# shichaoy/pop_up_slam

Measured on AMD Instinct MI355X. Metric: graph-solve iters/sec + final chi2, 1k-pose/5k-edge plane graph, higher is better.
Workload: dtype f64; 1 GPU; C2 synthetic corridor: 1000 SE3 poses, 200 planes, 5000 plane edges, 999 odometry edges (BASELINE.json configs[1], seed 42); jacobian_mode=numeric, total_lm_solves=773

## Files before the change

### pop_up_slam_amd/csrc/pps_k3.hip

```cpp
#include <algorithm>
#include <atomic>
#include <cstdlib>

#include <hip/hip_ext.h>

#include "pps_kcommon.h"
#include "pps_regtile.h"
#include "pps_front_reg.h"

namespace pps {



int lds_front_limit() {
  int fa = 1;
  while ((size_t)(fa + 1) * ((fa + 1) | 1) * 8 <= (size_t)kLdsLaunchCeilingBytes) fa++;
  return fa - 1;
}

template <bool USE_LDS>
__global__ __launch_bounds__(256) void k_front_factor(DevGraph d, int level_begin, double lambda) {
  extern __shared__ double lds[];
  const int s = d.level_fronts[level_begin + blockIdx.x];
  const int p = d.f_p[s], b = d.f_b[s];
// ... 207 lines not shown
#pragma unroll
    for (int r = 0; r < 4; r++) {
      cok[t][r] = rok[r] && br <= I + lq + 4 * r;
      const double craw = F[cok[t][r] ? crt[r] + br : 0];
      c[t][r] = cok[t][r] ? craw : 0.0;
    }
  }
#pragma unroll
  for (int t = 0; t < NT; t++) c[t] = __builtin_amdgcn_mfma_f64_16x16x4f64(av, bv[t], c[t], 0, 0, 0);
#pragma unroll
  for (int t = 0; t < NT; t++) {
    const int cc = o + 16 * t + l16;
#pragma unroll
    for (int r = 0; r < 4; r++)
      if (cok[t][r]) F[crt[r] + cc] = c[t][r];
  }
}

__device__ __forceinline__ void wave_front_factor(const DevGraph& d, int s_in, double lambda, double* __restrict__ F) {
  const int lane = threadIdx.x & 63;
  const int s = uni(s_in);
  const int p = uni(d.f_p[s]), b = uni(d.f_b[s]);
  const int f = p + b, fa = f + 1;
  const int ntri = tri(fa);
  PPS_TR(0);
  for (int i = lane; i < ntri; i += 64) F[i] = 0.0;
  __builtin_amdgcn_wave_barrier();
  PPS_TR(1);
  {
    const int e0 = uni(d.f_el_off[s]), e1 = uni(d.f_el_off[s + 1]);
    const double damp = 1.0 + lambda;
    const int* __restrict__ tgp = d.el_tgt;
    const double* __restrict__ hf = d.Hf;
    for (int e = e0 + lane; e < e1; e += 64 * 8) {
      int tg[8]; double v[8];
#pragma unroll
      for (int u = 0; u < 8; u++) { const int x = e + 64 * u; tg[u] = x < e1 ? tgp[x] : -1; v[u] = x < e1 ? hf[x] : 0.0; }
#pragma unroll
      for (int u = 0; u < 8; u++)
        if (tg[u] >= 0) F[tg[u] & 0x3fffffff] += (tg[u] & (1 << 30)) ? v[u] * damp : v[u];
    }
  }
  __builtin_amdgcn_wave_barrier();
  PPS_TR(2);
  const int ci0 = uni(d.f_child_off[s]), ci1 = uni(d.f_child_off[s + 1]);
  for (int ci = ci0; ci < ci1; ci++) {
    const int c = uni(d.child[ci]);
    const int bc1 = uni(d.f_b[c]) + 1;
    const int n = tri(bc1);
    const double* __restrict__ Uc = d.U + uni64(d.f_Uoff[c]);
    const int* __restrict__ tgc = d.ea_tgt + uni64(d.f_ea_off[c]);
    for (int e = lane; e < n; e += 64 * 8) {
      int tg[8]; double v[8];
#pragma unroll
      for (int u = 0; u < 8; u++) { const int x = e + 64 * u; tg[u] = x < n ? tgc[x] : -1; v[u] = x < n ? Uc[x] : 0.0; }
#pragma unroll
      for (int u = 0; u < 8; u++)
        if (tg[u] >= 0) F[tg[u]] += v[u];
    }
    __builtin_amdgcn_wave_barrier();
  }
  PPS_TR(3);
  const int r0 = lane, r1 = lane + 64;
  const int t0 = tri(r0), t1 = tri(r1);
  long long cyc_panel = 0, cyc_trail = 0;
  for (int K = 0; K < p; K += 4) {
    const long long tk0 = d.trace ? clock64() : 0;
    double a0[4], a1[4];
#pragma unroll
    for (int m = 0; m < 4; m++) {
      const int c = K + m;
      const bool v0 = c < p && r0 >= c && r0 < fa, v1 = c < p && r1 >= c && r1 < fa;
      const double x0 = F[v0 ? t0 + c : 0], x1 = F[v1 ? t1 + c : 0];
      a0[m] = v0 ? x0 : 0.0;
      a1[m] = v1 ? x1 : 0.0;
    }
#pragma unroll
    for (int m = 0; m < 4; m++) {
      const int c = K + m;
      if (c < p) {
        const double dmm = (c < 64) ? readlane_d(a0[m], c) : readlane_d(a1[m], c - 64);
        double dinv = 0.0;
        if (dmm > 0.0) dinv = rsqrt_nr(dmm);
        else if (lane == 0) raise_status(&d.result_dev[2], 1.0);
        if (r0 >= c) a0[m] *= dinv;
        if (r1 >= c) a1[m] *= dinv;
#pragma unroll
        for (int n = m + 1; n < 4; n++) {
          const int cn = K + n;
          if (cn < p) {
            const double lnm = (cn < 64) ? readlane_d(a0[m], cn) : readlane_d(a1[m], cn - 64);
            if (r0 >= cn) a0[n] -= a0[m] * lnm;
            if (r1 >= cn) a1[n] -= a1[m] * lnm;
          }
        }
      }
    }
#pragma unroll
    for (int m = 0; m < 4; m++) {
      const int c = K + m;
      if (c < p) {
        if (r0 >= c && r0 < fa) F[t0 + c] = a0[m];
        if (r1 >= c && r1 < fa) F[t1 + c] = a1[m];
      }
    }
    __builtin_amdgcn_wave_barrier();
    const long long tk1 = d.trace ? clock64() : 0;
    const int o = K + 4 < p ? K + 4 : p;
    const int nb = o - K;
    for (int I = o; I < fa; I += 16) {
      const int nt = ((I - o) >> 4) + 1;
      switch (nt) {
        case 1: trailing_tile_row<1>(F, fa, o, I, K, nb, lane); break;
        case 2: trailing_tile_row<2>(F, fa, o, I, K, nb, lane); break;
        case 3: trailing_tile_row<3>(F, fa, o, I, K, nb, lane); break;
        case 4: trailing_tile_row<4>(F, fa, o, I, K, nb, lane); break;
        case 5: trailing_tile_row<5>(F, fa, o, I, K, nb, lane); break;
        case 6: trailing_tile_row<6>(F, fa, o, I, K, nb, lane); break;
        case 7: trailing_tile_row<7>(F, fa, o, I, K, nb, lane); break;
        default: trailing_tile_row<8>(F, fa, o, I, K, nb, lane); break;
      }
    }
    __builtin_amdgcn_wave_barrier();
    if (d.trace) { const long long tk2 = clock64(); cyc_panel += tk1 - tk0; cyc_trail += tk2 - tk1; }
  }
  PPS_TR(4);
  if (d.trace && lane == 0) { d.trace[(size_t)s * 8 + 6] = cyc_panel; d.trace[(size_t)s * 8 + 7] = cyc_trail; }
  double* __restrict__ Lp = d.L + uni64(d.f_Loff[s]);
  if (lane < p) {
    for (int i0 = 0; i0 < fa; i0 += 8) {
      double v[8];
#pragma unroll
      for (int u = 0; u < 8; u++) { const int i = i0 + u; v[u] = F[(i < fa && lane <= i) ? tri(i) + lane : 0]; }
#pragma unroll
      for (int u = 0; u < 8; u++) { const int i = i0 + u; if (i < fa && lane <= i) Lp[(size_t)i * p + lane] = v[u]; }
    }
  }
  double* __restrict__ Us = d.U + uni64(d.f_Uoff[s]);
  for (int i0 = p; i0 < fa; i0 += 8) {
    for (int j = p + lane; j < fa; j += 64) {
      double v[8];
#pragma unroll
      for (int u = 0; u < 8; u++) { const int i = i0 + u; v[u] = F[(i < fa && j <= i) ? tri(i) + j : 0]; }
#pragma unroll
      for (int u = 0; u < 8; u++) { const int i = i0 + u; if (i < fa && j <= i) Us[tri(i - p) + j - p] = v[u]; }
    }
  }
  PPS_TR(5);
}

constexpr int kEaDepth = 10;
__device__ __forceinline__ void xg_store(double* p, double v) { __hip_atomic_store(p, v, __ATOMIC_RELAXED, __HIP_MEMORY_SCOPE_AGENT); }
__device__ __forceinline__ double xg_load(const double* p) { return __hip_atomic_load(p, __ATOMIC_RELAXED, __HIP_MEMORY_SCOPE_AGENT); }
template <int N> struct ElBatch { int tg[N]; double v[N]; };
template <int N, bool XH = false>
__device__ __forceinline__ void el_issue(const int* __restrict__ tgp, const double* __restrict__ val, int e, int e1, int lane, ElBatch<N>& q) {
  const int last = e1 > 0 ? e1 - 1 : 0;
#pragma unroll
  for (int u = 0; u < N; u++) {
    const int x = e + lane + 64 * u, xc = x < e1 ? x : last;
    const int t = tgp[xc];
    double v;
    if constexpr (XH) v = xg_load(val + xc); else v = val[xc];
    q.tg[u] = x < e1 ? t : -1; q.v[u] = x < e1 ? v : 0.0;
  }
}
template <bool ORIG, int N>
__device__ __forceinline__ void el_apply(const ElBatch<N>& q, double damp, double* __restrict__ F, int tr) {
  if constexpr (ORIG) {
#pragma unroll
    for (int u = 0; u < N; u++) {
      const int t = q.tg[u] >= 0 ? (q.tg[u] & 0x3fffffff) : tr;
      F[t] = (q.tg[u] & (1 << 30)) && q.tg[u] >= 0 ? q.v[u] * damp : q.v[u];
    }
    return;
  }
  int t[N]; double old[N];
#pragma unroll
  for (int u = 0; u < N; u++) { t[u] = q.tg[u] >= 0 ? q.tg[u] : tr; old[u] = F[t[u]]; }
#pragma unroll
  for (int u = 0; u < N; u++) F[t[u]] = old[u] + q.v[u];
}
template <int NPRE> struct FrontPre { ElBatch<NPRE> q; int crv; };
template <int NPRE>
__device__ __forceinline__ void front_pre_issue(const DevGraph& d, int rec, int lane, FrontPre<NPRE>& o) {
  const int e0 = __builtin_amdgcn_readlane(rec, 3), e1 = __builtin_amdgcn_readlane(rec, 4);
  const int cr0 = __builtin_amdgcn_readlane(rec, 5), nch = __builtin_amdgcn_readlane(rec, 6);
  el_issue(d.el_tgt, d.Hf, e0, e1, lane, o.q);
  o.crv = (lane < 8 * nch) ? d.crec[(size_t)cr0 * 8 + lane] : 0;
}
__device__ __forceinline__ void front_clear(int rec, int lane, double* __restrict__ F) {
  const int ntri = tri(__builtin_amdgcn_readlane(rec, 1) + __builtin_amdgcn_readlane(rec, 2) + 1);
  double2* __restrict__ F2 = reinterpret_cast<double2*>(F);
  const int n2 = ntri >> 1;
#pragma unroll 4
  for (int i = lane; i < n2; i += 64) F2[i] = make_double2(0.0, 0.0);
  if (lane == 0) F[ntri - 1] = 0.0;
  __builtin_amdgcn_wave_barrier();
}
template <int NPRE>
__device__ __forceinline__ void front_pre_finish(const DevGraph& d, int rec, int lane, const FrontPre<NPRE>& o, double damp, double* __restrict__ F, int tr) {
  const int e0 = __builtin_amdgcn_readlane(rec, 3), e1 = __builtin_amdgcn_readlane(rec, 4);
  el_apply<true>(o.q, damp, F, tr);
  for (int e = e0 + 64 * NPRE; e < e1; e += 64 * 8) { ElBatch<8> q; el_issue(d.el_tgt, d.Hf, e, e1, lane, q); __builtin_amdgcn_wave_barrier(); el_apply<true>(q, damp, F, tr); }
  __builtin_amdgcn_wave_barrier();
}
struct XGroup { int* flag; int epoch; double* hand; };
constexpr size_t kXgLdsFloorBytes = 82 * 1024;
__device__ __forceinline__ void xg_post(const XGroup& x, int s) {
  asm volatile("s_waitcnt vmcnt(0)" ::: "memory");
  if ((threadIdx.x & 63) == 0) __hip_atomic_store(x.flag + s, x.epoch, __ATOMIC_RELAXED, __HIP_MEMORY_SCOPE_AGENT);
}
template <bool ACQ>
__device__ __forceinline__ void xg_wait(const DevGraph& d, const XGroup& x, int s) {
  int spin = 0;
  while (__hip_atomic_load(x.flag + s, __ATOMIC_RELAXED, __HIP_MEMORY_SCOPE_AGENT) != x.epoch) {
    if (++spin >= (1 << 21)) { if ((threadIdx.x & 63) == 0) raise_status(&d.result_dev[2], kStatusInternal); break; }
    __builtin_amdgcn_s_sleep(2);
  }
  if (ACQ) __builtin_amdgcn_fence(__ATOMIC_ACQUIRE, "agent"); else __builtin_amdgcn_fence(__ATOMIC_ACQUIRE, "wavefront");
}
template <bool XG = false>
__device__ __forceinline__ void front_extend_add(const DevGraph& d, int rec, int crv0, int lane, double* __restrict__ F, int tr, const XGroup* xg = nullptr) {
  const int cr0 = __builtin_amdgcn_readlane(rec, 5), nch = __builtin_amdgcn_readlane(rec, 6);
  for (int cb = 0; cb < nch; cb += 8) {
    const int crv = cb == 0 ? crv0 : ((lane < 8 * (nch - cb)) ? d.crec[(size_t)(cr0 + cb) * 8 + lane] : 0);
    auto child = [&](int cj, int& n, const double* __restrict__& Uc, const int* __restrict__& tgc) {
      n = __builtin_amdgcn_readlane(crv, 8 * cj);
      const long long uo = ((long long)__builtin_amdgcn_readlane(crv, 8 * cj + 2) << 32) | (unsigned int)__builtin_amdgcn_readlane(crv, 8 * cj + 1);
      const long long eo = ((long long)__builtin_amdgcn_readlane(crv, 8 * cj + 4) << 32) | (unsigned int)__builtin_amdgcn_readlane(crv, 8 * cj + 3);
      Uc = d.U + uo; tgc = d.ea_tgt + eo;
    };
    int cj = 0;
    for (; cj < 8 && cb + cj < nch; cj++) {
      int n; const double* Uc; const int* tgc;
      child(cj, n, Uc, tgc);
      if (XG && __builtin_amdgcn_readlane(crv, 8 * cj + 6)) {
        xg_wait<false>(d, *xg, __builtin_amdgcn_readlane(crv, 8 * cj + 5));
        for (int e = 0; e < n; e += 64 * kEaDepth) { ElBatch<kEaDepth> q; el_issue<kEaDepth, true>(tgc, Uc, e, n, lane, q); __builtin_amdgcn_wave_barrier(); el_apply<false>(q, 0.0, F, tr); }
      } else
      for (int e = 0; e < n; e += 64 * kEaDepth) { ElBatch<kEaDepth> q; el_issue(tgc, Uc, e, n, lane, q); __builtin_amdgcn_wave_barrier(); el_apply<false>(q, 0.0, F, tr); }
      __builtin_amdgcn_wave_barrier();
    }
  }
}

constexpr int kPanelWBand = 4;
constexpr int kPanelWLevel = 8;
constexpr int kPanelWWide = 8;
template <bool TR>
__device__ __forceinline__ void front_assemble(const DevGraph& d, int rec, double lambda, double* F, int tr) {
  const int lane = threadIdx.x & 63;
  const int s = __builtin_amdgcn_readlane(rec, 0);
  (void)s;
  if (TR) PPS_TR(0);
  FrontPre<8> pre;
  front_pre_issue(d, rec, lane, pre);
  front_clear(rec, lane, F);
  if (TR) PPS_TR(1);
  front_pre_finish(d, rec, lane, pre, 1.0 + lambda, F, tr);
  if (TR) PPS_TR(2);
  front_extend_add(d, rec, pre.crv, lane, F, tr);
  if (TR) PPS_TR(3);
}
template <int NT, bool TR, bool STRIP = false, int W = kPanelWBand, bool XH = false>
__device__ __forceinline__ void front_eliminate_out(const DevGraph& d, int rec, double* F, double* P) {
  front_reg_eliminate<NT, TR, STRIP, W, XH>(d, rec, F, P);
}
template <int NT, bool TR, bool STRIP = false, int W = kPanelWBand>
__device__ __forceinline__ void wave_front_factor_reg(const DevGraph& d, int rec, double lambda, double* F, double* P, int tr) {
  front_assemble<TR>(d, rec, lambda, F, tr);
  front_eliminate_out<NT, TR, STRIP, W>(d, rec, F, P);
}

template <int K> __device__ __forceinline__ double row_bcast_d(double v) {
  int lo = __double2loint(v), hi = __double2hiint(v);
  lo = __builtin_amdgcn_update_dpp(0, lo, 0x150 + K, 0xf, 0xf, false);
  hi = __builtin_amdgcn_update_dpp(0, hi, 0x150 + K, 0xf, 0xf, false);
  return __hiloint2double(hi, lo);
}

constexpr double kFlowTimeout = kStatusInternal;
__device__ __forceinline__ void flow_wait(const DevGraph& d, int* flow, int q) {
  int spin = 0;
  while (__hip_atomic_load(flow + q, __ATOMIC_RELAXED, __HIP_MEMORY_SCOPE_WORKGROUP) == 0) {
    if (++spin >= (1 << 22)) { if ((threadIdx.x & 63) == 0) raise_status(&d.result_dev[2], kFlowTimeout); break; }
    __builtin_amdgcn_s_sleep(1);
  }
  __builtin_amdgcn_fence(__ATOMIC_ACQUIRE, "workgroup", "local");
}
__device__ __forceinline__ void flow_post(const DevGraph& d, int* flow, int slot, bool top) {
  __builtin_amdgcn_fence(__ATOMIC_RELEASE, "workgroup", "local");
  if ((threadIdx.x & 63) == 0 && !((d.sw & SW_DEBUG_DROP_FLAG) && top))
    __hip_atomic_store(flow + slot, 1, __ATOMIC_RELAXED, __HIP_MEMORY_SCOPE_WORKGROUP);
}

__device__ __forceinline__ bool xg_has_external_child(int rec, int crv, int lane) {
  const int nch = __builtin_amdgcn_readlane(rec, 6);
  return nch > 8 || __ballot((lane & 7) == 6 && lane < 8 * nch && crv != 0) != 0;
}
__device__ __forceinline__ void xg_publish(const XGroup& x, int s, int p, int b, int lane, double tj, double g0, double g1) {
  double* Xh = x.hand + (size_t)s * kBandMaxRows;
  if (lane < p) xg_store(Xh + lane, tj);
  if (lane < b) xg_store(Xh + p + lane, g0);
  if (lane + 64 < b) xg_store(Xh + p + lane + 64, g1);
  xg_post(x, s);
}

__device__ __forceinline__ void solve_pivot_scale(double (&lk)[16], double dinv) {
#define PPS_SC(U) lk[U] *= row_bcast_d<U>(dinv);
    PPS_SC(1) PPS_SC(2) PPS_SC(3) PPS_SC(4) PPS_SC(5) PPS_SC(6) PPS_SC(7) PPS_SC(8) PPS_SC(9) PPS_SC(10) PPS_SC(11) PPS_SC(12) PPS_SC(13) PPS_SC(14) PPS_SC(15)
#undef PPS_SC
}
template <bool SCALED = false>
__device__ __forceinline__ void solve_pivot_chain(int p, double (&lk)[16], double dinv, double& tj) {
#ifndef PPS_NO_FMA
#pragma clang fp contract(fast)
#endif
    if (!SCALED) solve_pivot_scale(lk, dinv);
#define PPS_BS(U) case U: tj -= lk[U] * row_bcast_d<U>(tj); [[fallthrough]];
    switch (p < 16 ? p - 1 : 15) {
      PPS_BS(15) PPS_BS(14) PPS_BS(13) PPS_BS(12) PPS_BS(11) PPS_BS(10) PPS_BS(9) PPS_BS(8)
      PPS_BS(7) PPS_BS(6) PPS_BS(5) PPS_BS(4) PPS_BS(3) PPS_BS(2)
      case 1: tj -= lk[1] * row_bcast_d<1>(tj); [[fallthrough]];
      default: break;
    }
#undef PPS_BS
    tj *= dinv;
}

template <bool GROUP = true, bool TR = false, bool XG = false>
__device__ __forceinline__ void wave_front_solve(const DevGraph& d, int rec, double* __restrict__ W, double* __restrict__ X, int slot, int* flow = nullptr, const XGroup* xg = nullptr) {
  const int lane = threadIdx.x & 63;
  const int s = __builtin_amdgcn_readlane(rec, 0);
  (void)s;
  if (TR) PPS_TR(0);
  const int p = __builtin_amdgcn_readlane(rec, 1), b = __builtin_amdgcn_readlane(rec, 2), f = p + b;
  const double* __restrict__ Lp = d.L + (((long long)__builtin_amdgcn_readlane(rec, 10) << 32) | (unsigned int)__builtin_amdgcn_readlane(rec, 9));
  const int pslot = GROUP ? __builtin_amdgcn_readlane(rec, 14) : -1;
  const int xpar = XG ? __builtin_amdgcn_readlane(rec, 13) : -1;
  int xcv = 0;
  if (XG) {
    const int nch = __builtin_amdgcn_readlane(rec, 6);
    const int* __restrict__ cp = nch > 0 ? d.crec + (size_t)__builtin_amdgcn_readlane(rec, 5) * 8 : d.frec;
    xcv = cp[lane < 8 * (nch < 8 ? nch : 8) ? lane : 0];
  }
  const int* __restrict__ ix = b == 0 ? d.frec : (pslot >= 0 || xpar >= 0 ? d.cmap + __builtin_amdgcn_readlane(rec, 15) : d.bidx + __builtin_amdgcn_readlane(rec, 8));
  double* xb = W;
  double* PL = W + kBandMaxRows;
  const int ix0r = ix[lane < b ? lane : 0], ix1r = ix[lane + 64 < b ? lane + 64 : 0];
  const int pix = d.pidx[__builtin_amdgcn_readlane(rec, 7) + (lane < p ? lane : 0)];
  const int n = (f + 1) * p;
  double tj = 0.0, dinv = 0.0;
  double lk[16];
  if (GROUP && p <= 16) {
#ifndef PPS_NO_FMA
#pragma clang fp contract(fast)
#endif
    const int j = lane & 15, part = lane >> 4;
    const int jc = j < p ? j : 0, lc = lane < p ? lane : 0;
    const double* __restrict__ LB = Lp + p * p + jc;
    const int blast = b > 0 ? b - 1 : 0;
    double lbv[12];
#pragma unroll
    for (int u = 0; u < 12; u++) { const int i = part + 4 * u; lbv[u] = LB[(i < b ? i : blast) * p]; }
#pragma unroll
    for (int u = 0; u < 16; u++) { const double l = Lp[(u < p ? u : p - 1) * p + lc]; lk[u] = lane < u ? l : 0.0; }
    const double dg = Lp[lc * p + lc], yr = Lp[f * p + jc];
    const int ix0 = lane < b ? ix0r : 0, ix1 = lane + 64 < b ? ix1r : 0;
    double g0 = 0.0, g1 = 0.0;
    const bool xpost = XG && xg_has_external_child(rec, xcv, lane);
    if (pslot < 0 && xpar < 0) { g0 = d.delta[ix0]; g1 = d.delta[ix1]; }
    if (flow) { dinv = 1.0 / dg; solve_pivot_scale(lk, dinv); }
    if (pslot >= 0) {
      if (flow) flow_wait(d, flow, pslot);
      const double* __restrict__ Xp = X + (size_t)pslot * kBandMaxRows; g0 = Xp[ix0]; g1 = Xp[ix1];
    } else if constexpr (XG) {
      if (xpar >= 0) {
        xg_wait<true>(d, *xg, xpar);
        const double* __restrict__ Xh = xg->hand + (size_t)xpar * kBandMaxRows; g0 = xg_load(Xh + ix0); g1 = xg_load(Xh + ix1);
      }
    }
    if (TR) PPS_TR(1);
    if (lane < b) xb[lane] = g0;
    if (lane + 64 < b) xb[lane + 64] = g1;
    __builtin_amdgcn_wave_barrier();
    if (TR) PPS_TR(2);
    if (!flow) dinv = 1.0 / dg;
    double a[4] = {part == 0 ? yr : 0.0, 0.0, 0.0, 0.0};
#pragma unroll
    for (int u = 0; u < 12; u++) { const int i = part + 4 * u; const double x = i < b ? xb[i] : 0.0; a[u & 3] -= lbv[u] * x; }
    for (int i0 = 48; i0 < b; i0 += 48) {
#pragma unroll
      for (int u = 0; u < 12; u++) { const int i = i0 + part + 4 * u; lbv[u] = LB[(i < b ? i : blast) * p]; }
// ... 83 lines not shown
      dinv = 1.0 / PL[lc * p + lc];
    }
    const int W = p <= 16 ? 16 : (p <= 32 ? 32 : 64), sh = p <= 16 ? 4 : (p <= 32 ? 5 : 6);
    const int j = lane & (W - 1), part = lane >> sh, np = 64 >> sh;
    const int jc = j < p ? j : 0;
    double a0 = (part == 0) ? (pre32 ? yq : PL[f * p + jc]) : 0.0, a1 = 0.0, a2 = 0.0, a3 = 0.0;
    const double* __restrict__ lb = PL + p * p + jc;
    int i_from = part;
    if (pre32) {
#pragma unroll
      for (int u = 0; u < 12; u += 4) {
        const int i = part + np * u, i1 = i + np, i2 = i + 2 * np, i3 = i + 3 * np;
        const double x0 = i < b ? xb[i] : 0.0, x1 = i1 < b ? xb[i1] : 0.0, x2 = i2 < b ? xb[i2] : 0.0, x3 = i3 < b ? xb[i3] : 0.0;
        if (i < b) { a0 -= lbq[u] * x0; a1 -= lbq[u + 1] * x1; a2 -= lbq[u + 2] * x2; a3 -= lbq[u + 3] * x3; }
      }
      i_from = part + 12 * np;
    }
    for (int i = i_from; i < b; i += 4 * np) {
      const int i1 = i + np, i2 = i + 2 * np, i3 = i + 3 * np;
      const double l0 = lb[i * p], l1 = lb[(i1 < b ? i1 : i) * p], l2 = lb[(i2 < b ? i2 : i) * p], l3 = lb[(i3 < b ? i3 : i) * p];
      const double x0 = xb[i], x1 = i1 < b ? xb[i1] : 0.0, x2 = i2 < b ? xb[i2] : 0.0, x3 = i3 < b ? xb[i3] : 0.0;
      a0 -= l0 * x0; a1 -= l1 * x1; a2 -= l2 * x2; a3 -= l3 * x3;
    }
    tj = (a0 + a1) + (a2 + a3);
    if (W <= 32) tj += __shfl_xor(tj, 32);
    if (W == 16) tj += __shfl_xor(tj, 16);
    tj = lane < p ? tj : 0.0;
    if (TR) PPS_TR(3);
    for (; k0 >= 16; k0 -= 16) {
#pragma unroll
      for (int u = 15; u >= 0; u--) {
        const int k = k0 + u;
        if (k < p) tj -= (pre_scaled ? lk[u] : lk[u] * readlane_d(dinv, k)) * readlane_d(tj, k);
      }
      pre_scaled = false;
#pragma unroll
      for (int u = 0; u < 16; u++) { const int k = k0 - 16 + u; const double l = PL[k * p + lc]; lk[u] = lane < k ? l : 0.0; }
    }
    solve_pivot_chain(p, lk, dinv, tj);
  }
  if (TR) PPS_TR(4);
  if (lane < p) d.delta[pix] = tj;
  if (TR) PPS_TR(5);
  if (!GROUP) return;
  double* __restrict__ Xs = X + (size_t)slot * kBandMaxRows;
  if (lane < p) Xs[lane] = tj;
  if (lane < b) Xs[p + lane] = g0;
  if (lane + 64 < b) Xs[p + lane + 64] = g1;
  if (flow) flow_post(d, flow, slot, pslot < 0);
  if (XG) { if (xpost) xg_publish(*xg, s, p, b, lane, tj, g0, g1); }
}

template <bool TR = false, bool XG = false>
__device__ __forceinline__ void body_band_solve_flow(const DevGraph& d, int g, int lds_doubles_per_wave, double* __restrict__ lds, int mg, const XGroup* xg = nullptr) {
  const int wave = uni(threadIdx.x >> 6), nw = blockDim.x >> 6;
  double* W = lds + (size_t)wave * lds_doubles_per_wave;
  double* X = lds + (size_t)nw * lds_doubles_per_wave;
  int* flow = reinterpret_cast<int*>(X + (size_t)mg * kBandMaxRows);
  const int2 span = reinterpret_cast<const int2*>(d.grp_span)[4 * (size_t)g];
  const int g0 = uni(span.x), gn = uni(span.y);
  const int i_first = g0 + gn - 1 - wave;
  int rec = i_first >= g0 ? d.frec[(size_t)i_first * 16 + (threadIdx.x & 15)] : 0;
  for (int q = threadIdx.x; q < gn; q += blockDim.x) flow[q] = 0;
  __syncthreads();
  for (int i = i_first; i >= g0; i -= nw) {
    wave_front_solve<true, TR, XG>(d, rec, W, X, i - g0, flow, xg);
    if (i - nw >= g0) rec = d.frec[(size_t)(i - nw) * 16 + (threadIdx.x & 15)];
  }
}
template <bool TR = false>
__device__ __forceinline__ void body_band_solve(const DevGraph& d, int g, int lds_doubles_per_wave, double* __restrict__ lds) {
  const int wave = uni(threadIdx.x >> 6), nw = blockDim.x >> 6;
  double* W = lds + (size_t)wave * lds_doubles_per_wave;
  double* X = lds + (size_t)nw * lds_doubles_per_wave;
  const int l0 = uni(d.grp_lvl_off[g]), l1 = uni(d.grp_lvl_off[g + 1]);
  int off[5], r4[4];
  {
    const int4 ga = reinterpret_cast<const int4*>(d.grp_span)[2 * (size_t)g], gb = reinterpret_cast<const int4*>(d.grp_span)[2 * (size_t)g + 1];
    off[0] = uni(ga.x); off[1] = uni(ga.w); off[2] = uni(gb.x); off[3] = uni(gb.y); off[4] = uni(gb.z);
  }
  const int g0 = off[0];
#pragma unroll
  for (int k = 0; k < 4; k++) { const int i = off[k] + wave; r4[k] = d.frec[(size_t)(i < off[k + 1] ? i : g0) * 16 + (threadIdx.x & 15)]; }
  for (int l = l1 - 1; l >= l0; l--) {
    const int k = l - l0;
    const int i0 = k < 4 ? (k == 3 ? off[3] : k == 2 ? off[2] : k == 1 ? off[1] : off[0]) : uni(d.glvl_front_off[l]);
    const int i1 = k < 4 ? (k == 3 ? off[4] : k == 2 ? off[3] : k == 1 ? off[2] : off[1]) : uni(d.glvl_front_off[l + 1]);
    for (int i = i0 + wave; i < i1; i += nw) {
      const int rec = (k < 4 && i == i0 + wave) ? (k == 3 ? r4[3] : k == 2 ? r4[2] : k == 1 ? r4[1] : r4[0]) : d.frec[(size_t)i * 16 + (threadIdx.x & 15)];
      wave_front_solve<true, TR>(d, rec, W, X, i - g0);
    }
    asm volatile("s_waitcnt lgkmcnt(0)\n\ts_barrier" ::: "memory");
  }
}

template <bool RESULT = true>
__device__ __forceinline__ void take_alt(DevGraph& d, const DualAlt& a) {
  if (blockIdx.y) { d.L = a.L; d.U = a.U; d.delta = a.delta; if (RESULT) d.result_dev = a.result_dev; }
}
__device__ __forceinline__ void take_alt(DevGraph& d, const DualAlt& a, double& lambda) {
  if (blockIdx.y) { d.L = a.L; d.U = a.U; d.delta = a.delta; d.result_dev = a.result_dev; lambda = a.lambda; }
}
__global__ __launch_bounds__(512) void k_band_solve(DevGraph d, DualAlt alt, int grp_begin, int lds_doubles_per_wave) {
  extern __shared__ double lds[];
  take_alt<false>(d, alt);
  body_band_solve(d, grp_begin + blockIdx.x, lds_doubles_per_wave, lds);
}
__global__ __launch_bounds__(768) void k_band_solve_flow(DevGraph d, DualAlt alt, int grp_begin, int lds_doubles_per_wave, int mg) {
  extern __shared__ double lds[];
  take_alt(d, alt);
  body_band_solve_flow(d, grp_begin + blockIdx.x, lds_doubles_per_wave, lds, mg);
}
__global__ __launch_bounds__(768) void k_band_solve_flow_trace(DevGraph d, int grp_begin, int lds_doubles_per_wave, int mg) {
  extern __shared__ double lds[];
  body_band_solve_flow<true>(d, grp_begin + blockIdx.x, lds_doubles_per_wave, lds, mg);
}
__global__ __launch_bounds__(512) void k_band_solve_trace(DevGraph d, int grp_begin, int lds_doubles_per_wave) {
  extern __shared__ double lds[];
  body_band_solve<true>(d, grp_begin + blockIdx.x, lds_doubles_per_wave, lds);
}

template <bool REG_ONLY, bool REG_STRIP = false, bool TR = false, bool R5 = false>
__device__ __forceinline__ void body_band_factor(const DevGraph& d, int g, double lambda, int lds_doubles_per_wave, double* __restrict__ lds) {
  const int wave = uni(threadIdx.x >> 6), nw = blockDim.x >> 6;
  double* F = lds + (size_t)wave * lds_doubles_per_wave;
  const int l0 = d.grp_lvl_off[g], l1 = d.grp_lvl_off[g + 1];
  const int4 ga = reinterpret_cast<const int4*>(d.grp_span)[2 * (size_t)g];
  for (int l = l0; l < l1; l++) {
    const int i1 = l == l0 ? ga.w : d.glvl_front_off[l + 1];
    for (int i = (l == l0 ? ga.x : d.glvl_front_off[l]) + wave; i < i1; i += nw) {
      const int rec = d.frec[(size_t)i * 16 + (threadIdx.x & 15)];
      const int s = __builtin_amdgcn_readlane(rec, 0);
      const int fa = __builtin_amdgcn_readlane(rec, 1) + __builtin_amdgcn_readlane(rec, 2) + 1;
      constexpr bool ALIAS = REG_ONLY && !REG_STRIP;
      double* const Pn = ALIAS ? F : F + lds_doubles_per_wave - kRegRowsMax * kP8Stride;
      const int tr = ALIAS ? lds_doubles_per_wave - 1 : lds_doubles_per_wave - kRegRowsMax * kP8Stride - 1;
      constexpr int WB = kPanelWBand, WR = kPanelWWide;
      if (REG_ONLY || fa <= kRegRowsMax) {
        if (REG_ONLY) front_assemble<TR>(d, rec, lambda, F, tr);
        else if ((fa <= kRegRowsMax && !d.no_strip) || fa <= kRegRows) front_assemble<true>(d, rec, lambda, F, tr);
      }
      if (REG_ONLY && fa <= 33) front_eliminate_out<2, TR, false, REG_STRIP ? WR : WB>(d, rec, F, Pn);
      else if (REG_ONLY && fa <= 49) front_eliminate_out<3, TR, false, REG_STRIP ? WR : WB>(d, rec, F, Pn);
      else if (REG_ONLY && (!REG_STRIP || fa <= kRegRows)) front_eliminate_out<4, TR, false, REG_STRIP ? WR : WB>(d, rec, F, Pn);
      else if (REG_ONLY && R5) front_eliminate_out<5, false, true, WR>(d, rec, F, Pn);
      else if (fa <= kRegRowsMax && !d.no_strip) front_eliminate_out<4, true, true, WR>(d, rec, F, Pn);
      else if (fa <= kRegRows) front_eliminate_out<4, true, false, WR>(d, rec, F, Pn);
      else wave_front_factor(d, s, lambda, F);
    }
    __syncthreads();
  }
}

template <int NPRE>
__device__ __forceinline__ int front_orig_entries(const DevGraph& d, int rec, int lane, double damp, double* F, int tr) {
  FrontPre<NPRE> pre;
  front_pre_issue(d, rec, lane, pre);
  front_clear(rec, lane, F);
  front_pre_finish(d, rec, lane, pre, damp, F, tr);
  return pre.crv;
}
__device__ __forceinline__ int front_orig_entries_sized(const DevGraph& d, int rec, int lane, double damp, double* F, int tr) {
  const int n_el = __builtin_amdgcn_readlane(rec, 4) - __builtin_amdgcn_readlane(rec, 3);
  if (n_el <= 192) return front_orig_entries<3>(d, rec, lane, damp, F, tr);
  return front_orig_entries<8>(d, rec, lane, damp, F, tr);
}

template <bool XG = false>
__device__ __forceinline__ void body_band_factor_pre(const DevGraph& d, int g, double lambda, int lds_doubles_per_wave, double* __restrict__ lds, const XGroup* xg = nullptr) {
  const int wave = uni(threadIdx.x >> 6), lane = threadIdx.x & 63, nw = uni(blockDim.x >> 6);
  const int4 ga = reinterpret_cast<const int4*>(d.grp_span)[2 * (size_t)g], gb = reinterpret_cast<const int4*>(d.grp_span)[2 * (size_t)g + 1];
  const int nl = uni(ga.z);
  const int o0 = uni(ga.x), o1 = uni(ga.w), o2 = uni(gb.x), o3 = uni(gb.y), o4 = uni(gb.z);
  const int n0 = o1 - o0, n1 = nl > 1 ? o2 - o1 : 0, n2 = nl > 2 ? o3 - o2 : 0, n3 = nl > 3 ? o4 - o3 : 0;
  double* F = lds + (size_t)wave * lds_doubles_per_wave;
  const int tr = lds_doubles_per_wave - 1;
  const bool shape_b = n0 + n1 + n2 + n3 <= nw;
  const int b1 = shape_b ? n0 : 0, b2 = shape_b ? n0 + n1 : n1, b3 = b2 + n2;
  int up_ll = 0, up_rec = 0;
  {
    int up_i = 0;
    if (shape_b && wave >= b1 && wave < b1 + n1) { up_ll = 1; up_i = o1 + wave - b1; }
    else if (wave >= b2 && wave < b2 + n2 && (shape_b || wave >= n1)) { up_ll = 2; up_i = o2 + wave - b2; }
    else if (wave >= b3 && wave < b3 + n3) { up_ll = 3; up_i = o3 + wave - b3; }
    if (up_ll) up_rec = d.frec[(size_t)up_i * 16 + (threadIdx.x & 15)];
  }
  const int pre_at = shape_b ? 0 : 1;
  int crv = 0;
  for (int ll = 0; ll < nl; ll++) {
    const int lb = ll == 0 ? 0 : ll == 1 ? b1 : ll == 2 ? b2 : b3;
    const int cnt = ll == 0 ? n0 : ll == 1 ? n1 : ll == 2 ? n2 : n3;
    const int i0 = ll == 0 ? o0 : ll == 1 ? o1 : ll == 2 ? o2 : o3;
    const bool mine = wave >= lb && wave < lb + cnt;
    const bool mine_up = mine && up_ll == ll && ll > pre_at;
    if (mine) {
      const int rec = (up_ll == ll && ll > 0) ? up_rec : d.frec[(size_t)(i0 + wave - lb) * 16 + (threadIdx.x & 15)];
      const int fa = __builtin_amdgcn_readlane(rec, 1) + __builtin_amdgcn_readlane(rec, 2) + 1;
      if (!mine_up) crv = front_orig_entries_sized(d, rec, lane, 1.0 + lambda, F, tr);
      front_extend_add<XG>(d, rec, crv, lane, F, tr, xg);
      if (fa <= 33) front_eliminate_out<2, false, false, kPanelWBand, XG>(d, rec, F, F);
      else if (fa <= 49) front_eliminate_out<3, false, false, kPanelWBand, XG>(d, rec, F, F);
      else front_eliminate_out<4, false, false, kPanelWBand, XG>(d, rec, F, F);
      if (XG) { if (__builtin_amdgcn_readlane(rec, 13) >= 0 && !(d.sw & SW_DEBUG_DROP_XFLAG)) xg_post(*xg, __builtin_amdgcn_readlane(rec, 0)); }
    } else if (ll == pre_at && up_ll > pre_at) {
      crv = front_orig_entries_sized(d, up_rec, lane, 1.0 + lambda, F, tr);
    }
    __syncthreads();
  }
}

template <bool REG_ONLY>
__global__ __launch_bounds__(512) void k_band_factor(DevGraph d, DualAlt alt, int grp_begin, double lambda, int lds_doubles_per_wave) {
  extern __shared__ double lds[];
  if (blockIdx.y) { d.L = alt.L; d.U = alt.U; d.delta = alt.delta; d.result_dev = alt.result_dev; lambda = alt.lambda; }
  body_band_factor<REG_ONLY>(d, grp_begin + blockIdx.x, lambda, lds_doubles_per_wave, lds);
}

template <bool PRE, bool FLOW>
__global__ __launch_bounds__(512) void k_band_root(DevGraph d, DualAlt alt, int grp, double lambda, int per_wave_factor, int per_wave_solve, int mg) {
  extern __shared__ double lds[];
  if (blockIdx.y) { d.L = alt.L; d.U = alt.U; d.delta = alt.delta; d.result_dev = alt.result_dev; lambda = alt.lambda; }
  if (PRE) body_band_factor_pre(d, grp, lambda, per_wave_factor, lds); else body_band_factor<true>(d, grp, lambda, per_wave_factor, lds);
  if (FLOW) body_band_solve_flow(d, grp, per_wave_solve, lds, mg); else body_band_solve(d, grp, per_wave_solve, lds);
}

__global__ __launch_bounds__(512) void k_band_factor_all(DevGraph d, DualAlt alt, double lambda, int lds_doubles_per_wave, int epoch) {
  extern __shared__ double lds[];
  XGroup xg{d.k3_flag, epoch, nullptr};
  if (blockIdx.y) { d.L = alt.L; d.U = alt.U; d.delta = alt.delta; d.result_dev = alt.result_dev; lambda = alt.lambda; xg.flag += d.n_fronts; }
  body_band_factor_pre<true>(d, blockIdx.x, lambda, lds_doubles_per_wave, lds, &xg);
}
__global__ __launch_bounds__(768) void k_band_solve_all(DevGraph d, DualAlt alt, int n_groups, int lds_doubles_per_wave, int mg, int epoch) {
  extern __shared__ double lds[];
  XGroup xg{d.k3_flag + 2 * d.n_fronts, epoch, d.k3_xhand};
  if (blockIdx.y) { d.L = alt.L; d.U = alt.U; d.delta = alt.delta; d.result_dev = alt.result_dev; xg.flag += d.n_fronts; xg.hand += (size_t)d.n_fronts * kBandMaxRows; }
  body_band_solve_flow<false, true>(d, n_groups - 1 - (int)blockIdx.x, lds_doubles_per_wave, lds, mg, &xg);
}

__global__ __launch_bounds__(512) void k_band_factor_pre(DevGraph d, DualAlt alt, int grp_begin, double lambda, int lds_doubles_per_wave) {
  extern __shared__ double lds[];
  take_alt(d, alt, lambda);
  body_band_factor_pre(d, grp_begin + blockIdx.x, lambda, lds_doubles_per_wave, lds);
}

__global__ __launch_bounds__(512) void k_band_factor_lean_trace(DevGraph d, DualAlt alt, int grp_begin, double lambda, int lds_doubles_per_wave) {
  extern __shared__ double lds[];
  body_band_factor<true, false, true>(d, grp_begin + blockIdx.x, lambda, lds_doubles_per_wave, lds);
}

__global__ __launch_bounds__(256) __attribute__((amdgpu_waves_per_eu(1, 1)))
void k_band_factor_r5(DevGraph d, DualAlt alt, int grp_begin, double lambda, int lds_doubles_per_wave) {
  extern __shared__ double lds[];
  take_alt(d, alt, lambda);
  body_band_factor<true, true, false, true>(d, grp_begin + blockIdx.x, lambda, lds_doubles_per_wave, lds);
}

static inline DualAlt alt_arg(const DualAlt* alt) { return alt ? *alt : DualAlt{}; }

hipError_t launch_band_factor(const DevGraph& d, const DualAlt* alt, const K3StagePlan& sp, double lambda, hipStream_t st, hipEvent_t ev0, hipEvent_t ev1,
                              bool pre_ok) {
  if (sp.grp_count == 0) return hipSuccess;
  const bool reg = sp.reg_only && !(alt && d.trace != nullptr), r5 = !reg && sp.r5_ok;
  const auto kernel = reg ? (d.trace != nullptr ? &k_band_factor_lean_trace : sp.pre && pre_ok ? &k_band_factor_pre : &k_band_factor<true>)
                          : (r5 ? &k_band_factor_r5 : &k_band_factor<false>);
  PPS_LAUNCH_EV(ev0, ev1, kernel, dim3(sp.grp_count, alt ? 2 : 1), dim3(64 * (r5 ? sp.nw_factor_r5 : sp.nw_factor)),
                reg ? sp.lds_factor_reg : r5 ? sp.lds_factor_r5 : sp.lds_factor_gen, st, d, alt_arg(alt), sp.grp_begin, lambda, reg ? sp.pw_factor_reg : sp.pw_factor_gen);
  return hipGetLastError();
}

hipError_t launch_band_solve(const DevGraph& d, const DualAlt* alt, const K3StagePlan& sp, hipStream_t st) {
  if (sp.grp_count == 0) return hipSuccess;
  const bool trace = d.trace != nullptr && d.trace_solve;
  const dim3 grid(sp.grp_count, alt ? 2 : 1);
  if (sp.nw_flow > 0 && !(trace && alt)) {
    if (trace) PPS_LAUNCH(k_band_solve_flow_trace, dim3(sp.grp_count), dim3(64 * sp.nw_flow), sp.lds_flow, st, d, sp.grp_begin, sp.pw_solve, sp.max_grp_fronts);
    else PPS_LAUNCH(k_band_solve_flow, grid, dim3(64 * sp.nw_flow), sp.lds_flow, st, d, alt_arg(alt), sp.grp_begin, sp.pw_solve, sp.max_grp_fronts);
  }
  else if (trace && !alt) PPS_LAUNCH(k_band_solve_trace, dim3(sp.grp_count), dim3(64 * sp.nw_solve), sp.lds_solve, st, d, sp.grp_begin, sp.pw_solve);
  else PPS_LAUNCH(k_band_solve, grid, dim3(64 * sp.nw_solve), sp.lds_solve, st, d, alt_arg(alt), sp.grp_begin, sp.pw_solve);
  return hipGetLastError();
}

hipError_t launch_band_root(const DevGraph& d, const DualAlt* alt, const K3Plan& p, double lambda, hipStream_t st, hipEvent_t ev0, hipEvent_t ev1) {
  const K3RootPlan& r = p.root;
  const int grp = p.stages.back().grp_begin;
  const dim3 grid(1, alt ? 2 : 1), block(64 * r.nw);
  const DualAlt a2 = alt_arg(alt);
  const auto kernel = r.pre ? (r.flow ? &k_band_root<true, true> : &k_band_root<true, false>) : (r.flow ? &k_band_root<false, true> : &k_band_root<false, false>);
  PPS_LAUNCH_EV(ev0, ev1, kernel, grid, block, r.lds, st, d, a2, grp, lambda, r.pw_factor, r.pw_solve, r.max_grp_fronts);
  return hipGetLastError();
}

hipError_t launch_band_all_factor(const DevGraph& d, const DualAlt* alt, const K3Plan& p, double lambda, int epoch, hipStream_t st, hipEvent_t ev0,
                                  hipEvent_t ev1) {
  const K3AllPlan& a = p.all;
  PPS_LAUNCH_EV(ev0, ev1, k_band_factor_all, dim3(a.n_groups, alt ? 2 : 1), dim3(64 * a.nw_factor), std::max(a.lds_factor, kXgLdsFloorBytes), st, d, alt_arg(alt), lambda, a.pw_factor, epoch);
  return hipGetLastError();
}
hipError_t launch_band_all_solve(const DevGraph& d, const DualAlt* alt, const K3Plan& p, int epoch, hipStream_t st) {
  const K3AllPlan& a = p.all;
  PPS_LAUNCH(k_band_solve_all, dim3(a.n_groups, alt ? 2 : 1), dim3(64 * a.nw_solve), std::max(a.lds_solve, kXgLdsFloorBytes), st, d, alt_arg(alt), a.n_groups, a.pw_solve, a.max_grp_fronts, epoch);
  return hipGetLastError();
}

__global__ __launch_bounds__(64) void k_front_solve(DevGraph d, int level_begin) {
  __shared__ double t[256];
  const int s = d.level_fronts[level_begin + blockIdx.x];
  const int p = d.f_p[s], b = d.f_b[s], f = p + b;
  const double* __restrict__ Lp = d.L + d.f_Loff[s];
  const int* __restrict__ bi = d.bidx + d.f_bidx_off[s];
  const int lane = threadIdx.x;
  for (int k = lane; k < p; k += 64) {
    double acc = Lp[(size_t)f * p + k];
    for (int i = 0; i < b; i++) acc -= Lp[(size_t)(p + i) * p + k] * d.delta[bi[i]];
    t[k] = acc;
  }
  __syncthreads();
  for (int k = p - 1; k >= 0; k--) {
    const double xk = t[k] / Lp[(size_t)k * p + k];
    __syncthreads();
    for (int j = lane; j < k; j += 64) t[j] -= Lp[(size_t)k * p + j] * xk;
    if (lane == 0) t[k] = xk;
    __syncthreads();
  }
  for (int k = lane; k < p; k += 64) d.delta[d.pidx[d.f_poff[s] + k]] = t[k];
}

hipError_t launch_backsolve_level(const DevGraph& d, int level_begin, int level_count, hipStream_t st) {
  if (level_count == 0) return hipSuccess;
  PPS_LAUNCH(k_front_solve, dim3(level_count), dim3(64), 0, st, d, level_begin);
  return hipGetLastError();
}

template <bool REG_ONLY>
__global__ __launch_bounds__(512) void kb_band_factor(BatchArgs a, int stage, int lds_doubles_per_wave) {
  extern __shared__ double lds[];
  PPS_BATCH_PROLOGUE(BF_ACTIVE)
  const BatchStage sg = a.stage_tab[(size_t)stage * a.n_total + a.b0 + b];
  if ((int)blockIdx.x >= sg.grp_count) return;
  DevGraph d2 = d;
  double lam = a.lambda[b];
  if (blockIdx.z) {
    const BatchAlt al = load_alt(a.alt + a.b0 + b);
    d2.L = al.L; d2.U = al.U; d2.delta = al.delta; d2.result_dev = al.result_dev;
    lam = a.lambda2[b];
  }
  body_band_factor<REG_ONLY>(d2, sg.grp_begin + blockIdx.x, lam, lds_doubles_per_wave, lds);
}

__global__ __launch_bounds__(512) void kb_band_factor_pre(BatchArgs a, int stage, int lds_doubles_per_wave) {
  extern __shared__ double lds[];
  PPS_BATCH_PROLOGUE(BF_ACTIVE)
  const BatchStage sg = a.stage_tab[(size_t)stage * a.n_total + a.b0 + b];
  if ((int)blockIdx.x >= sg.grp_count) return;
  DevGraph d2 = d;
  double lam = a.lambda[b];
  if (blockIdx.z) {
    const BatchAlt al = load_alt(a.alt + a.b0 + b);
    d2.L = al.L; d2.U = al.U; d2.delta = al.delta; d2.result_dev = al.result_dev;
    lam = a.lambda2[b];
  }
// ... 286 lines not shown
```

Baseline: 18550 LM iters/s.

## Prefetch child extend-add targets across level barrier and pair two-child fronts

Splits element-list loads into separate target-index and value loads and replaces the per-entry sentinel with a per-lane count. For fronts with exactly two children, the wave that will process the front at the next level prefetches both children's target indices before the level barrier. It then issues both children's value loads together so their latencies overlap. It also widens the original-entry prefetch to 11 batches for large fronts, skips the tail loop when the prefetch already covers everything, and moves the per-level barrier. This adds register pressure and reorders barriers, which risks occupancy loss or a correctness issue if the barrier move breaks inter-level dependencies.

```diff
diff --git a/pop_up_slam_amd/csrc/pps_k3.hip b/pop_up_slam_amd/csrc/pps_k3.hip
--- a/pop_up_slam_amd/csrc/pps_k3.hip
+++ b/pop_up_slam_amd/csrc/pps_k3.hip
@@ -383,34 +383,40 @@
 constexpr int kEaDepth = 10;
 __device__ __forceinline__ void xg_store(double* p, double v) { __hip_atomic_store(p, v, __ATOMIC_RELAXED, __HIP_MEMORY_SCOPE_AGENT); }
 __device__ __forceinline__ double xg_load(const double* p) { return __hip_atomic_load(p, __ATOMIC_RELAXED, __HIP_MEMORY_SCOPE_AGENT); }
-template <int N> struct ElBatch { int tg[N]; double v[N]; };
+template <int N> struct ElBatch { int tg[N]; double v[N]; int cnt; };
+__device__ __forceinline__ int el_clamp(int e, int e1, int lane, int u) { const int x = e + lane + 64 * u, last = e1 > 0 ? e1 - 1 : 0; return x < e1 ? x : last; }
+template <int N>
+__device__ __forceinline__ void el_issue_tgt(const int* __restrict__ tgp, int e, int e1, int lane, int (&tg)[N]) {
+#pragma unroll
+  for (int u = 0; u < N; u++) tg[u] = tgp[el_clamp(e, e1, lane, u)];
+}
+template <int N, bool XH = false>
+__device__ __forceinline__ void el_issue_val(const double* __restrict__ val, int e, int e1, int lane, ElBatch<N>& q) {
+#pragma unroll
+  for (int u = 0; u < N; u++) { const int xc = el_clamp(e, e1, lane, u); if constexpr (XH) q.v[u] = xg_load(val + xc); else q.v[u] = val[xc]; }
+  q.cnt = e1 - e - lane;
+}
 template <int N, bool XH = false>
 __device__ __forceinline__ void el_issue(const int* __restrict__ tgp, const double* __restrict__ val, int e, int e1, int lane, ElBatch<N>& q) {
-  const int last = e1 > 0 ? e1 - 1 : 0;
-#pragma unroll
-  for (int u = 0; u < N; u++) {
-    const int x = e + lane + 64 * u, xc = x < e1 ? x : last;
-    const int t = tgp[xc];
-    double v;
-    if constexpr (XH) v = xg_load(val + xc); else v = val[xc];
-    q.tg[u] = x < e1 ? t : -1; q.v[u] = x < e1 ? v : 0.0;
-  }
+  el_issue_tgt(tgp, e, e1, lane, q.tg);
+  el_issue_val<N, XH>(val, e, e1, lane, q);
 }
 template <bool ORIG, int N>
 __device__ __forceinline__ void el_apply(const ElBatch<N>& q, double damp, double* __restrict__ F, int tr) {
   if constexpr (ORIG) {
 #pragma unroll
     for (int u = 0; u < N; u++) {
-      const int t = q.tg[u] >= 0 ? (q.tg[u] & 0x3fffffff) : tr;
-      F[t] = (q.tg[u] & (1 << 30)) && q.tg[u] >= 0 ? q.v[u] * damp : q.v[u];
+      const bool ex = 64 * u < q.cnt;
+      const double v = (q.tg[u] & (1 << 30)) ? q.v[u] * damp : q.v[u];
+      F[ex ? (q.tg[u] & 0x3fffffff) : tr] = ex ? v : 0.0;
     }
     return;
   }
   int t[N]; double old[N];
 #pragma unroll
-  for (int u = 0; u < N; u++) { t[u] = q.tg[u] >= 0 ? q.tg[u] : tr; old[u] = F[t[u]]; }
-#pragma unroll
-  for (int u = 0; u < N; u++) F[t[u]] = old[u] + q.v[u];
+  for (int u = 0; u < N; u++) { t[u] = 64 * u < q.cnt ? q.tg[u] : tr; old[u] = F[t[u]]; }
+#pragma unroll
+  for (int u = 0; u < N; u++) F[t[u]] = old[u] + (64 * u < q.cnt ? q.v[u] : 0.0);
 }
 template <int NPRE> struct FrontPre { ElBatch<NPRE> q; int crv; };
 template <int NPRE>
@@ -429,11 +435,12 @@
   if (lane == 0) F[ntri - 1] = 0.0;
   __builtin_amdgcn_wave_barrier();
 }
-template <int NPRE>
+template <int NPRE, bool TAIL = true>
 __device__ __forceinline__ void front_pre_finish(const DevGraph& d, int rec, int lane, const FrontPre<NPRE>& o, double damp, double* __restrict__ F, int tr) {
   const int e0 = __builtin_amdgcn_readlane(rec, 3), e1 = __builtin_amdgcn_readlane(rec, 4);
   el_apply<true>(o.q, damp, F, tr);
-  for (int e = e0 + 64 * NPRE; e < e1; e += 64 * 8) { ElBatch<8> q; el_issue(d.el_tgt, d.Hf, e, e1, lane, q); __builtin_amdgcn_wave_barrier(); el_apply<true>(q, damp, F, tr); }
+  if constexpr (TAIL)
+    for (int e = e0 + 64 * NPRE; e < e1; e += 64 * 8) { ElBatch<8> q; el_issue(d.el_tgt, d.Hf, e, e1, lane, q); __builtin_amdgcn_wave_barrier(); el_apply<true>(q, damp, F, tr); }
   __builtin_amdgcn_wave_barrier();
 }
 struct XGroup { int* flag; int epoch; double* hand; };
@@ -451,26 +458,59 @@
   }
   if (ACQ) __builtin_amdgcn_fence(__ATOMIC_ACQUIRE, "agent"); else __builtin_amdgcn_fence(__ATOMIC_ACQUIRE, "wavefront");
 }
-template <bool XG = false>
-__device__ __forceinline__ void front_extend_add(const DevGraph& d, int rec, int crv0, int lane, double* __restrict__ F, int tr, const XGroup* xg = nullptr) {
+struct EaChild { int n; const double* U; const int* tg; };
+__device__ __forceinline__ EaChild ea_child(const DevGraph& d, int crv, int cj) {
+  const long long uo = ((long long)__builtin_amdgcn_readlane(crv, 8 * cj + 2) << 32) | (unsigned int)__builtin_amdgcn_readlane(crv, 8 * cj + 1);
+  const long long eo = ((long long)__builtin_amdgcn_readlane(crv, 8 * cj + 4) << 32) | (unsigned int)__builtin_amdgcn_readlane(crv, 8 * cj + 3);
+  return {__builtin_amdgcn_readlane(crv, 8 * cj), d.U + uo, d.ea_tgt + eo};
+}
+struct EaPre { int tg[2][kEaDepth]; };
+__device__ __forceinline__ bool ea_pairable(int rec, int crv) {
+  return __builtin_amdgcn_readlane(rec, 6) == 2 && __builtin_amdgcn_readlane(crv, 0) > 0 && __builtin_amdgcn_readlane(crv, 8) > 0;
+}
+__device__ __forceinline__ void ea_pre_issue(const DevGraph& d, int crv, int lane, EaPre& o) {
+#pragma unroll
+  for (int c = 0; c < 2; c++) { const EaChild ch = ea_child(d, crv, c); el_issue_tgt(ch.tg, 0, ch.n, lane, o.tg[c]); }
+}
+template <bool XG = false, bool PAIR = false>
+__device__ __forceinline__ void front_extend_add(const DevGraph& d, int rec, int crv0, int lane, double* __restrict__ F, int tr, const XGroup* xg = nullptr,
+                                                 const EaPre* pre = nullptr, bool have_pre = false) {
   const int cr0 = __builtin_amdgcn_readlane(rec, 5), nch = __builtin_amdgcn_readlane(rec, 6);
+  auto batches = [&](const EaChild& c, int e0, bool xh) {
+    if (XG && xh) for (int e = e0; e < c.n; e += 64 * kEaDepth) { ElBatch<kEaDepth> q; el_issue<kEaDepth, true>(c.tg, c.U, e, c.n, lane, q); __builtin_amdgcn_wave_barrier(); el_apply<false>(q, 0.0, F, tr); }
+    else for (int e = e0; e < c.n; e += 64 * kEaDepth) { ElBatch<kEaDepth> q; el_issue(c.tg, c.U, e, c.n, lane, q); __builtin_amdgcn_wave_barrier(); el_apply<false>(q, 0.0, F, tr); }
+  };
+  if constexpr (PAIR) {
+    const bool xh0 = XG && __builtin_amdgcn_readlane(crv0, 6), xh1 = XG && __builtin_amdgcn_readlane(crv0, 14);
+    if (ea_pairable(rec, crv0) && (have_pre || xh0 || xh1)) {
+      ElBatch<kEaDepth> q[2];
+      if (have_pre) {
+#pragma unroll
+        for (int u = 0; u < kEaDepth; u++) { q[0].tg[u] = pre->tg[0][u]; q[1].tg[u] = pre->tg[1][u]; }
+      }
+      const EaChild c0 = ea_child(d, crv0, 0), c1 = ea_child(d, crv0, 1);
+      if (!have_pre) { el_issue_tgt(c0.tg, 0, c0.n, lane, q[0].tg); el_issue_tgt(c1.tg, 0, c1.n, lane, q[1].tg); }
+      if (XG && xh0) { xg_wait<false>(d, *xg, __builtin_amdgcn_readlane(crv0, 5)); el_issue_val<kEaDepth, true>(c0.U, 0, c0.n, lane, q[0]); }
+      else el_issue_val(c0.U, 0, c0.n, lane, q[0]);
+      if (XG && xh1) { xg_wait<false>(d, *xg, __builtin_amdgcn_readlane(crv0, 13)); el_issue_val<kEaDepth, true>(c1.U, 0, c1.n, lane, q[1]); }
+      else el_issue_val(c1.U, 0, c1.n, lane, q[1]);
+      __builtin_amdgcn_wave_barrier();
+      el_apply<false>(q[0], 0.0, F, tr);
+      batches(c0, 64 * kEaDepth, xh0);
+      __builtin_amdgcn_wave_barrier();
+      el_apply<false>(q[1], 0.0, F, tr);
+      batches(c1, 64 * kEaDepth, xh1);
+      __builtin_amdgcn_wave_barrier();
+      return;
+    }
+  }
   for (int cb = 0; cb < nch; cb += 8) {
     const int crv = cb == 0 ? crv0 : ((lane < 8 * (nch - cb)) ? d.crec[(size_t)(cr0 + cb) * 8 + lane] : 0);
-    auto child = [&](int cj, int& n, const double* __restrict__& Uc, const int* __restrict__& tgc) {
-      n = __builtin_amdgcn_readlane(crv, 8 * cj);
-      const long long uo = ((long long)__builtin_amdgcn_readlane(crv, 8 * cj + 2) << 32) | (unsigned int)__builtin_amdgcn_readlane(crv, 8 * cj + 1);
-      const long long eo = ((long long)__builtin_amdgcn_readlane(crv, 8 * cj + 4) << 32) | (unsigned int)__builtin_amdgcn_readlane(crv, 8 * cj + 3);
-      Uc = d.U + uo; tgc = d.ea_tgt + eo;
-    };
-    int cj = 0;
-    for (; cj < 8 && cb + cj < nch; cj++) {
-      int n; const double* Uc; const int* tgc;
-      child(cj, n, Uc, tgc);
-      if (XG && __builtin_amdgcn_readlane(crv, 8 * cj + 6)) {
-        xg_wait<false>(d, *xg, __builtin_amdgcn_readlane(crv, 8 * cj + 5));
-        for (int e = 0; e < n; e += 64 * kEaDepth) { ElBatch<kEaDepth> q; el_issue<kEaDepth, true>(tgc, Uc, e, n, lane, q); __builtin_amdgcn_wave_barrier(); el_apply<false>(q, 0.0, F, tr); }
-      } else
-      for (int e = 0; e < n; e += 64 * kEaDepth) { ElBatch<kEaDepth> q; el_issue(tgc, Uc, e, n, lane, q); __builtin_amdgcn_wave_barrier(); el_apply<false>(q, 0.0, F, tr); }
+    for (int cj = 0; cj < 8 && cb + cj < nch; cj++) {
+      const EaChild c = ea_child(d, crv, cj);
+      const bool xh = XG && __builtin_amdgcn_readlane(crv, 8 * cj + 6);
+      if (XG && xh) xg_wait<false>(d, *xg, __builtin_amdgcn_readlane(crv, 8 * cj + 5));
+      batches(c, 0, xh);
       __builtin_amdgcn_wave_barrier();
     }
   }
@@ -860,18 +900,19 @@
   }
 }
 
-template <int NPRE>
+template <int NPRE, bool TAIL>
 __device__ __forceinline__ int front_orig_entries(const DevGraph& d, int rec, int lane, double damp, double* F, int tr) {
   FrontPre<NPRE> pre;
   front_pre_issue(d, rec, lane, pre);
   front_clear(rec, lane, F);
-  front_pre_finish(d, rec, lane, pre, damp, F, tr);
+  front_pre_finish<NPRE, TAIL>(d, rec, lane, pre, damp, F, tr);
   return pre.crv;
 }
 __device__ __forceinline__ int front_orig_entries_sized(const DevGraph& d, int rec, int lane, double damp, double* F, int tr) {
   const int n_el = __builtin_amdgcn_readlane(rec, 4) - __builtin_amdgcn_readlane(rec, 3);
-  if (n_el <= 192) return front_orig_entries<3>(d, rec, lane, damp, F, tr);
-  return front_orig_entries<8>(d, rec, lane, damp, F, tr);
+  if (n_el <= 192) return front_orig_entries<3, false>(d, rec, lane, damp, F, tr);
+  if (n_el <= 512) return front_orig_entries<8, false>(d, rec, lane, damp, F, tr);
+  return front_orig_entries<11, true>(d, rec, lane, damp, F, tr);
 }
 
 template <bool XG = false>
@@ -901,11 +942,17 @@
     const int i0 = ll == 0 ? o0 : ll == 1 ? o1 : ll == 2 ? o2 : o3;
     const bool mine = wave >= lb && wave < lb + cnt;
     const bool mine_up = mine && up_ll == ll && ll > pre_at;
+    EaPre eat; bool have_pre = false;
+    if (ll > 0) {
+      have_pre = mine_up && ea_pairable(up_rec, crv);
+      if (have_pre) ea_pre_issue(d, crv, lane, eat);
+      __syncthreads();
+    }
     if (mine) {
       const int rec = (up_ll == ll && ll > 0) ? up_rec : d.frec[(size_t)(i0 + wave - lb) * 16 + (threadIdx.x & 15)];
       const int fa = __builtin_amdgcn_readlane(rec, 1) + __builtin_amdgcn_readlane(rec, 2) + 1;
       if (!mine_up) crv = front_orig_entries_sized(d, rec, lane, 1.0 + lambda, F, tr);
-      front_extend_add<XG>(d, rec, crv, lane, F, tr, xg);
+      front_extend_add<XG, true>(d, rec, crv, lane, F, tr, xg, &eat, have_pre);
       if (fa <= 33) front_eliminate_out<2, false, false, kPanelWBand, XG>(d, rec, F, F);
       else if (fa <= 49) front_eliminate_out<3, false, false, kPanelWBand, XG>(d, rec, F, F);
       else front_eliminate_out<4, false, false, kPanelWBand, XG>(d, rec, F, F);
@@ -913,8 +960,8 @@
     } else if (ll == pre_at && up_ll > pre_at) {
       crv = front_orig_entries_sized(d, up_rec, lane, 1.0 + lambda, F, tr);
     }
-    __syncthreads();
-  }
+  }
+  __syncthreads();
 }
 
 template <bool REG_ONLY>
```

Result: faster. 18910 LM iters/s (median of 6 runs) (+2.0%).
